# submission2019/cnn-quantization

Hardware: NVIDIA H100
Metric: resnet50_w4a4_images_per_s (higher is better)
Workload: dtype f32

## Files before the change

### cnn-quantization_b200/csrc/fq_bulk.cuh

```cuda
#pragma once
#include <cuda_runtime.h>
#include <stdint.h>

#include "fq_device.cuh"

namespace fqb {

constexpr int kConsumers = kThreads;
constexpr int kBulkThreads = kConsumers + 32;
constexpr int kConsumerWarps = kConsumers / 32;
#ifndef FQB_STAGE_VEC
#define FQB_STAGE_VEC 4
#endif
#ifndef FQB_STAGES
#define FQB_STAGES 6
#endif
#ifndef FQB_BULK_CTAS
#define FQB_BULK_CTAS 1
#endif
constexpr int kBulkCtasPerSm = FQB_BULK_CTAS;
constexpr int kStageVec = FQB_STAGE_VEC;
constexpr int kStages = FQB_STAGES;
constexpr unsigned kStageBytes = kStageVec * kConsumers * 16u;
#ifndef FQB_BULK_SPLIT
// ... 47 lines not shown
  unsigned stride;
  unsigned stage_v;
  unsigned n_stages;
  unsigned unit_stages;
  unsigned units;
  unsigned channels;
  unsigned cv;
};

struct StageMeta {
  unsigned start;
  unsigned count;
  unsigned tag;
  unsigned pad;
};

struct BulkRing {
  alignas(8) unsigned long long full[kStages];
  alignas(8) unsigned long long empty[kStages];
  StageMeta meta[kStages];
  unsigned nstages;
};

struct RingPos {
  unsigned slot, parity, n;
  __device__ __forceinline__ void init(unsigned nstages = kStages) {
    slot = 0;
    parity = 0;
    n = nstages;
  }
  __device__ __forceinline__ void next() {
    if (++slot == n) {
      slot = 0;
      parity ^= 1u;
    }
  }
};

__device__ __forceinline__ void ring_init(BulkRing& r, unsigned nstages = kStages) {
  if (threadIdx.x == 0) {
    r.nstages = nstages;
#pragma unroll
    for (int s = 0; s < kStages; ++s) {
      mbar_init(smem_u32(&r.full[s]), 1u);
      mbar_init(smem_u32(&r.empty[s]), kConsumerWarps);
    }
    mbar_fence_init();
  }
  __syncthreads();
}

struct TicketPlan {
  unsigned nstatic;
  unsigned first, step;
  unsigned dyn_base;
};

constexpr unsigned kPairOffset = kStageBytes / 2u;

__device__ __forceinline__ FlatGeo half_geo(const FlatGeo& g) {
  FlatGeo h = g;
  h.stage_v = (kStageVec / 2u) * g.stride;
  h.n_stages = (g.total_v + h.stage_v - 1u) / h.stage_v;
  h.unit_stages = 2u * g.unit_stages;
  return h;
}

template <bool REV, bool PAIR = false>
__device__ __forceinline__ void produce_phase(const FlatGeo& g, const float4* src, unsigned* counter, const TicketPlan tp,
                                              BulkRing& r, unsigned char* stage_base, RingPos& pos,
                                              const float4* src2 = nullptr) {
  const unsigned total = g.units;
  unsigned k = 0;
  auto fetch = [&]() -> unsigned {
    unsigned long long t;
    if (k < tp.nstatic)
      t = tp.first + static_cast<unsigned long long>(k) * tp.step;
    else
      t = static_cast<unsigned long long>(tp.dyn_base) + atomicAdd(counter, 1u);
    ++k;
    return t < total ? static_cast<unsigned>(t) : 0xffffffffu;
  };
  unsigned cur = fetch();
  unsigned nxt = (cur != 0xffffffffu) ? fetch() : 0xffffffffu;
  while (cur != 0xffffffffu) {
    const unsigned nxt2 = (nxt != 0xffffffffu) ? fetch() : 0xffffffffu;
    const unsigned u = REV ? total - 1u - cur : cur;
    const unsigned g0 = u * g.unit_stages;
    const unsigned g1 = min(g0 + g.unit_stages, g.n_stages);
    for (unsigned i = g0; i < g1; ++i) {
      const unsigned st = REV ? g1 - 1u - (i - g0) : i;
      const unsigned start = st * g.stage_v;
      const unsigned count = min(g.stage_v, g.total_v - start);
      mbar_wait(smem_u32(&r.empty[pos.slot]), pos.parity ^ 1u);
      r.meta[pos.slot].start = start;
      r.meta[pos.slot].count = count;
      r.meta[pos.slot].tag = 0u;
      const unsigned bar = smem_u32(&r.full[pos.slot]);
      mbar_arrive_expect_tx(bar, PAIR ? count * 32u : count * 16u);
      bulk_load(smem_u32(stage_base + pos.slot * kStageBytes), src + start, count * 16u, bar);
      if (PAIR) bulk_load(smem_u32(stage_base + pos.slot * kStageBytes + kPairOffset), src2 + start, count * 16u, bar);
      pos.next();
    }
    cur = nxt;
    nxt = nxt2;
  }
  mbar_wait(smem_u32(&r.empty[pos.slot]), pos.parity ^ 1u);
  r.meta[pos.slot].start = 0u;
  r.meta[pos.slot].count = 0u;
  mbar_arrive(smem_u32(&r.full[pos.slot]));
  pos.next();
}

struct RowsGeo {
  unsigned rows, row_v;
  unsigned stages_per_row;
  unsigned units_per_row;
};

__device__ __forceinline__ RowsGeo half_rows(const FlatGeo& h, const RowsGeo& rg) {
  RowsGeo r = rg;
  r.stages_per_row = (rg.row_v + h.stage_v - 1u) / h.stage_v;
  r.units_per_row = (r.stages_per_row + h.unit_stages - 1u) / h.unit_stages;
  return r;
}

template <bool REV, bool PAIR = false>
__device__ __forceinline__ void produce_rows_phase(const FlatGeo& g, const RowsGeo& rg, const float4* src, unsigned* counter,
                                                   const TicketPlan tp, BulkRing& r, unsigned char* stage_base, RingPos& pos,
                                                   const float4* src2 = nullptr) {
  const unsigned total = g.units;
  unsigned k = 0;
  auto fetch = [&]() -> unsigned {
    unsigned long long t;
    if (k < tp.nstatic)
      t = tp.first + static_cast<unsigned long long>(k) * tp.step;
    else
      t = static_cast<unsigned long long>(tp.dyn_base) + atomicAdd(counter, 1u);
    ++k;
    return t < total ? static_cast<unsigned>(t) : 0xffffffffu;
  };
  unsigned cur = fetch();
  unsigned nxt = (cur != 0xffffffffu) ? fetch() : 0xffffffffu;
  while (cur != 0xffffffffu) {
    const unsigned nxt2 = (nxt != 0xffffffffu) ? fetch() : 0xffffffffu;
    const unsigned u = REV ? total - 1u - cur : cur;
    const unsigned row = u / rg.units_per_row;
    const unsigned part = u - row * rg.units_per_row;
    const unsigned s0 = part * g.unit_stages;
    const unsigned s1 = min(s0 + g.unit_stages, rg.stages_per_row);
    for (unsigned i = s0; i < s1; ++i) {
      const unsigned st = REV ? s1 - 1u - (i - s0) : i;
      const unsigned off = st * g.stage_v;
      const unsigned start = row * rg.row_v + off;
      const unsigned count = min(g.stage_v, rg.row_v - off);
      mbar_wait(smem_u32(&r.empty[pos.slot]), pos.parity ^ 1u);
      r.meta[pos.slot].start = start;
      r.meta[pos.slot].count = count;
      r.meta[pos.slot].tag = row | (i + 1u == s1 ? 0x80000000u : 0u);
      const unsigned bar = smem_u32(&r.full[pos.slot]);
      mbar_arrive_expect_tx(bar, PAIR ? count * 32u : count * 16u);
      bulk_load(smem_u32(stage_base + pos.slot * kStageBytes), src + start, count * 16u, bar);
      if (PAIR) bulk_load(smem_u32(stage_base + pos.slot * kStageBytes + kPairOffset), src2 + start, count * 16u, bar);
      pos.next();
    }
    cur = nxt;
    nxt = nxt2;
  }
  mbar_wait(smem_u32(&r.empty[pos.slot]), pos.parity ^ 1u);
  r.meta[pos.slot].start = 0u;
  r.meta[pos.slot].count = 0u;
  r.meta[pos.slot].tag = 0u;
  mbar_arrive(smem_u32(&r.full[pos.slot]));
  pos.next();
}

struct PoolGeo {
  unsigned h, w;
  unsigned wt;
  unsigned tiles_per_row;
  unsigned row_pairs;
  unsigned tiles;
  unsigned unit_tiles, units;
  unsigned ow;
  unsigned kind;
};

constexpr unsigned kPoolTop = 1u, kPoolLeft = 2u;

__device__ __forceinline__ void produce_pool3_phase(const FlatGeo& g, const PoolGeo& pg, const float4* src, unsigned* counter,
                                                    const TicketPlan tp, BulkRing& r, unsigned char* stage_base, RingPos& pos) {
  const unsigned total = pg.units;
  unsigned k = 0;
  auto fetch = [&]() -> unsigned {
    unsigned long long t;
    if (k < tp.nstatic)
      t = tp.first + static_cast<unsigned long long>(k) * tp.step;
    else
      t = static_cast<unsigned long long>(tp.dyn_base) + atomicAdd(counter, 1u);
    ++k;
    return t < total ? static_cast<unsigned>(t) : 0xffffffffu;
  };
  const unsigned row_v = pg.w * g.cv;
  const unsigned region_v = (2u * pg.wt + 1u) * g.cv;
  const unsigned per_img = pg.row_pairs * pg.tiles_per_row;
  unsigned cur = fetch();
  unsigned nxt = (cur != 0xffffffffu) ? fetch() : 0xffffffffu;
  while (cur != 0xffffffffu) {
    const unsigned nxt2 = (nxt != 0xffffffffu) ? fetch() : 0xffffffffu;
    const unsigned t0 = cur * pg.unit_tiles;
    const unsigned t1 = min(t0 + pg.unit_tiles, pg.tiles);
    for (unsigned tile = t0; tile < t1; ++tile) {
      const unsigned n = tile / per_img;
      const unsigned rem = tile - n * per_img;
      const unsigned oh = rem / pg.tiles_per_row;
      const unsigned wi = rem - oh * pg.tiles_per_row;
      const bool top = oh > 0u, left = wi > 0u;
      const unsigned skip = left ? 0u : g.cv;
      const unsigned count = region_v - skip;
      const unsigned mid = (n * pg.h + 2u * oh) * row_v + (2u * wi * pg.wt) * g.cv - (left ? g.cv : 0u);
      const unsigned o = ((n * pg.row_pairs + oh) * pg.ow + wi * pg.wt) * g.cv;
      mbar_wait(smem_u32(&r.empty[pos.slot]), pos.parity ^ 1u);
      r.meta[pos.slot].start = o;
      r.meta[pos.slot].count = count;
      r.meta[pos.slot].tag = (top ? kPoolTop : 0u) | (left ? kPoolLeft : 0u);
      const unsigned bar = smem_u32(&r.full[pos.slot]);
      mbar_arrive_expect_tx(bar, count * 16u * (top ? 3u : 2u));
      const unsigned dst = smem_u32(stage_base + pos.slot * kStageBytes) + skip * 16u;
      if (top) bulk_load(dst, src + mid - row_v, count * 16u, bar);
      bulk_load(dst + region_v * 16u, src + mid, count * 16u, bar);
      bulk_load(dst + 2u * region_v * 16u, src + mid + row_v, count * 16u, bar);
      pos.next();
    }
    cur = nxt;
    nxt = nxt2;
  }
  mbar_wait(smem_u32(&r.empty[pos.slot]), pos.parity ^ 1u);
  r.meta[pos.slot].start = 0u;
  r.meta[pos.slot].count = 0u;
  r.meta[pos.slot].tag = 0u;
  mbar_arrive(smem_u32(&r.full[pos.slot]));
  pos.next();
}

template <typename Acc>
__device__ __forceinline__ void consume_pool3_phase(const FlatGeo& g, const PoolGeo& pg, BulkRing& r, const unsigned char* stage_base,
                                                    RingPos& pos, Acc& acc) {
  const unsigned t = threadIdx.x;
  const bool lane0 = (t & 31u) == 0u;
  const bool mine = t < pg.wt * g.cv;
  const unsigned j = t / g.cv, col = t - j * g.cv;
  const unsigned region = (2u * pg.wt + 1u) * g.cv * 16u;
  const unsigned my = smem_u32(stage_base) + ((2u * j) * g.cv + col) * 16u;
  const unsigned nxt = g.cv * 16u;
  for (;;) {
    mbar_wait(smem_u32(&r.full[pos.slot]), pos.parity);
    const StageMeta m = r.meta[pos.slot];
    if (m.count != 0u && mine) {
      const unsigned addr = my + pos.slot * kStageBytes;
      const bool first = (j != 0u) || (m.tag & kPoolLeft);
      acc.pool_begin();
#pragma unroll
      for (int dy = 0; dy < 3; ++dy) {
        if (dy == 0 && !(m.tag & kPoolTop)) continue;
        const unsigned row = addr + dy * region;
        float4 v;
        if (first) {
          lds_vec(row, v);
          acc.pool_tap(v);
        }
        lds_vec(row + nxt, v);
        acc.pool_tap(v);
        lds_vec(row + 2u * nxt, v);
        acc.pool_tap(v);
      }
      acc.pool_end(m.start + t);
    }
    __syncwarp();
    if (lane0) mbar_arrive(smem_u32(&r.empty[pos.slot]));
    pos.next();
    if (m.count == 0u) break;
  }
}

__device__ __forceinline__ void produce_pool_phase(const FlatGeo& g, const PoolGeo& pg, const float4* src, unsigned* counter,
                                                   const TicketPlan tp, BulkRing& r, unsigned char* stage_base, RingPos& pos) {
  const unsigned total = pg.units;
  unsigned k = 0;
  auto fetch = [&]() -> unsigned {
    unsigned long long t;
    if (k < tp.nstatic)
      t = tp.first + static_cast<unsigned long long>(k) * tp.step;
    else
      t = static_cast<unsigned long long>(tp.dyn_base) + atomicAdd(counter, 1u);
    ++k;
    return t < total ? static_cast<unsigned>(t) : 0xffffffffu;
  };
  const unsigned row_v = pg.w * g.cv;
  const unsigned count = pg.wt * g.cv;
  const unsigned per_img = pg.row_pairs * pg.tiles_per_row;
  unsigned cur = fetch();
  unsigned nxt = (cur != 0xffffffffu) ? fetch() : 0xffffffffu;
  while (cur != 0xffffffffu) {
    const unsigned nxt2 = (nxt != 0xffffffffu) ? fetch() : 0xffffffffu;
    const unsigned t0 = cur * pg.unit_tiles;
    const unsigned t1 = min(t0 + pg.unit_tiles, pg.tiles);
    for (unsigned tile = t0; tile < t1; ++tile) {
      const unsigned n = tile / per_img;
      const unsigned rem = tile - n * per_img;
      const unsigned hp = rem / pg.tiles_per_row;
      const unsigned wi = rem - hp * pg.tiles_per_row;
      const unsigned a = (n * pg.h + 2u * hp) * row_v + wi * count;
      const unsigned o = ((n * pg.row_pairs + hp) * pg.ow + wi * (pg.wt / 2u)) * g.cv;
      mbar_wait(smem_u32(&r.empty[pos.slot]), pos.parity ^ 1u);
      r.meta[pos.slot].start = o;
      r.meta[pos.slot].count = count;
      r.meta[pos.slot].tag = 0u;
      const unsigned bar = smem_u32(&r.full[pos.slot]);
      mbar_arrive_expect_tx(bar, count * 32u);
      bulk_load(smem_u32(stage_base + pos.slot * kStageBytes), src + a, count * 16u, bar);
      bulk_load(smem_u32(stage_base + pos.slot * kStageBytes + kPairOffset), src + a + row_v, count * 16u, bar);
      pos.next();
    }
    cur = nxt;
    nxt = nxt2;
  }
  mbar_wait(smem_u32(&r.empty[pos.slot]), pos.parity ^ 1u);
  r.meta[pos.slot].start = 0u;
  r.meta[pos.slot].count = 0u;
  r.meta[pos.slot].tag = 0u;
  mbar_arrive(smem_u32(&r.full[pos.slot]));
  pos.next();
}

template <typename Acc>
__device__ __forceinline__ void consume_pool_phase(const FlatGeo& g, const PoolGeo& pg, BulkRing& r, const unsigned char* stage_base,
                                                   RingPos& pos, Acc& acc) {
  const unsigned t = threadIdx.x;
  const bool lane0 = (t & 31u) == 0u;
  const bool mine = t < (pg.wt / 2u) * g.cv;
  const unsigned j = t / g.cv, col = t - j * g.cv;
  const unsigned my = smem_u32(stage_base) + ((2u * j) * g.cv + col) * 16u;
  const unsigned nxt = g.cv * 16u;
  for (;;) {
    mbar_wait(smem_u32(&r.full[pos.slot]), pos.parity);
    const StageMeta m = r.meta[pos.slot];
    if (m.count != 0u && mine) {
      const unsigned addr = my + pos.slot * kStageBytes;
      float4 a0, a1, b0, b1;
      lds_vec(addr, a0);
      lds_vec(addr + nxt, a1);
      lds_vec(addr + kPairOffset, b0);
      lds_vec(addr + kPairOffset + nxt, b1);
      acc.pooled(a0, a1, b0, b1, m.start + t);
    }
    __syncwarp();
    if (lane0) mbar_arrive(smem_u32(&r.empty[pos.slot]));
    pos.next();
    if (m.count == 0u) break;
  }
}

template <typename Acc>
__device__ __forceinline__ void consume_phase(const FlatGeo& g, BulkRing& r, const unsigned char* stage_base, RingPos& pos,
                                              Acc& acc) {
  const unsigned t = threadIdx.x;
  const bool lane0 = (t & 31u) == 0u;
  const unsigned my = smem_u32(stage_base) + t * 16u;
  const unsigned step = g.stride * 16u;
  for (;;) {
    mbar_wait(smem_u32(&r.full[pos.slot]), pos.parity);
    const StageMeta m = r.meta[pos.slot];
    const unsigned addr = my + pos.slot * kStageBytes;
    if (m.count == g.stage_v) {
      if (t < g.stride) {
        float4 x[kStageVec];
#pragma unroll
        for (int i = 0; i < kStageVec; ++i) lds_vec(addr + i * step, x[i]);
#pragma unroll
        for (int i = 0; i < kStageVec; ++i) acc.consume(x[i], m.start + t + i * g.stride);
      }
    } else if (m.count != 0u) {
#pragma unroll
      for (int i = 0; i < kStageVec; ++i) {
        const unsigned idx = t + i * g.stride;
        if (t < g.stride && idx < m.count) {
          float4 x;
          lds_vec(addr + i * step, x);
          acc.consume(x, m.start + idx);
        }
      }
    }
    acc.stage_end(m);
    __syncwarp();
    if (lane0) mbar_arrive(smem_u32(&r.empty[pos.slot]));
    pos.next();
    if (m.count == 0u) break;
  }
}

template <typename Acc>
__device__ __forceinline__ void consume_pair_phase(const FlatGeo& g, BulkRing& r, const unsigned char* stage_base, RingPos& pos,
                                                   Acc& acc) {
  static_assert(kStageVec % 2u == 0u, "a pair stage is split in two halves");
  constexpr int kHalf = kStageVec / 2;
  const unsigned t = threadIdx.x;
  const bool lane0 = (t & 31u) == 0u;
  const unsigned my = smem_u32(stage_base) + t * 16u;
// ... 38 lines not shown
```

### cnn-quantization_b200/csrc/fq_cl.cuh

```cuda
#pragma once

namespace fqb {

__device__ __forceinline__ unsigned enc_ordered(float x) {
  const unsigned b = __float_as_uint(x);
  return (b & 0x80000000u) ? ~b : (b | 0x80000000u);
}
__device__ __forceinline__ float dec_ordered(unsigned e) {
  return __uint_as_float((e & 0x80000000u) ? (e & 0x7fffffffu) : ~e);
}

constexpr unsigned kAccU = 2u * kMaxNhwcChannels;
constexpr unsigned kAccD = 3u * kMaxNhwcChannels;

struct ClView {
  unsigned* amin_inv;
  unsigned* amax;
  double* asum;
  double* asq;
  double* aabs;
};
__device__ __forceinline__ ClView cl_view(const FusedArgs& A, unsigned bank) {
  ClView v;
  v.amin_inv = A.amin_inv + bank * kAccU;
// ... 635 lines not shown
      produce_phase<false>(g, src, &A.sync->unit_counter[0], all, ring, stages, pos);
      if (DEV) {
        mbar_wait(smem_u32(&phase_go[0]), 0u);
        if (solver_in_s2 && blockIdx.x == 0) mbar_wait(smem_u32(&solver_done), 0u);
        produce_phase<true>(g, src, &A.sync->unit_counter[1], solver_in_s2 ? no0 : all, ring, stages, pos);
      }
      if (!A.stats_only) {
        mbar_wait(smem_u32(&phase_go[1]), 0u);
        if (A.pool.tiles && A.pool.kind == 3u)
          produce_pool3_phase(g, A.pool, src, &A.sync->unit_counter[2], all, ring, stages, pos);
        else if (A.pool.tiles)
          produce_pool_phase(g, A.pool, src, &A.sync->unit_counter[2], all, ring, stages, pos);
        else if (A.residual)
          produce_phase<!DEV, true>(half_geo(g), src, &A.sync->unit_counter[2], all, ring, stages, pos,
                                    reinterpret_cast<const float4*>(A.residual));
        else
          produce_phase<!DEV>(g, src, &A.sync->unit_counter[2], all, ring, stages, pos);
      }
    }
    return;
  }

  const unsigned t = threadIdx.x;
  const bool active = t < g.stride;
  const bool direct = cv == g.stride;
  const unsigned col = active ? t % cv : 0u;
  const unsigned c0 = 4u * col;
  const double n = A.n_per_group;
  const ClView acc = cl_view(A, bank);
  const unsigned rep = A.nhwc_rep;
  const unsigned rep_base = (blockIdx.x % rep) * C;
  unsigned epoch = 0;
  if (blockIdx.x == 0) stamp(A, 0);

  if (blockIdx.x == gridDim.x - 1u) {
    const ClView other = cl_view(A, bank ^ 1u);
    uint4* zu = reinterpret_cast<uint4*>(other.amin_inv);
    uint4* zd = reinterpret_cast<uint4*>(other.asum);
    const uint4 z = make_uint4(0u, 0u, 0u, 0u);
    for (unsigned i = t; i < kAccU / 4u; i += kConsumers) zu[i] = z;
    for (unsigned i = t; i < kAccD / 2u; i += kConsumers) zd[i] = z;
  }

  ClCtx cx;
  cx.g = &g;
  cx.ring = &ring;
  cx.stages = stages;
  cx.cbuf = cbuf;
  cx.pos.init(nstages);
  cx.acc = acc;
  cx.rep_base = rep_base;
  cx.c0 = c0;
  cx.active = active;
  float kshift[4];
  cl_phase_s1(A, cx, kshift);
  if (t == 0) mbar_arrive(smem_u32(&phase_go[DEV ? 0 : 1]));
  if (blockIdx.x == 0) stamp(A, 1);
  grid_barrier_cl(A.sync, epoch);
  if (blockIdx.x == 0) stamp(A, 4);

  float mean[4];
  if (direct) {
#pragma unroll
    for (int i = 0; i < 4; ++i)
      mean[i] = static_cast<float>(cl_mean(acc, rep, C, c0 + i, kshift[i], (A.bias && active) ? __ldg(A.bias + c0 + i) : 0.f, n));
  } else {
    for (unsigned c = t; c < C; c += kConsumers)
      tab_mean[c] = static_cast<float>(cl_mean(acc, rep, C, c, ld_tensor(A.in + c), A.bias ? __ldg(A.bias + c) : 0.f, n));
    consumer_sync();
#pragma unroll
    for (int i = 0; i < 4; ++i) mean[i] = tab_mean[c0 + i];
  }

  if (alloc && !aux_needs_b && blockIdx.x == 0) {
    cl_solve_aux(A, acc, lsm, tag, false, !solver_in_s2);
    stamp(A, 12);
    if (t == 0) mbar_arrive(smem_u32(&solver_done));
  }

  if constexpr (DEV) {
    cl_phase_s2(A, cx, mean);
    if (t == 0) mbar_arrive(smem_u32(&phase_go[1]));
    if (blockIdx.x == 0) stamp(A, 5);
    grid_barrier_cl(A.sync, epoch);
    if (blockIdx.x == 0) stamp(A, 8);
    if (aux_needs_b && blockIdx.x == 0) cl_solve_aux(A, acc, lsm, tag, true, true);
  }
  if (alloc && !solver_in_s2) {
    if (t == 0)
      while (ld_acquire_u32(&A.sync->aux_ready) != tag) __nanosleep(40);
    consumer_sync();
  }

  LeafParam lp[4];
  const bool do_export = A.out_stats != nullptr && blockIdx.x == 0;
  if (direct) {
#pragma unroll
    for (int i = 0; i < 4; ++i) lp[i] = cl_channel_param<LEAF, DEV>(A, acc, rep, C, c0 + i, mean[i], n, alloc, do_export && active);
  } else {
    LeafParam* tab_lp = reinterpret_cast<LeafParam*>(cbuf);
    consumer_sync();
    for (unsigned c = t; c < C; c += kConsumers) tab_lp[c] = cl_channel_param<LEAF, DEV>(A, acc, rep, C, c, tab_mean[c], n, alloc, do_export);
    consumer_sync();
#pragma unroll
    for (int i = 0; i < 4; ++i) lp[i] = tab_lp[c0 + i];
  }
  if (blockIdx.x == 0) stamp(A, 7);

  if (!A.stats_only) {
    cl_phase_apply<LEAF, HIST>(A, cx, lp, hist);
    if (blockIdx.x == 0) stamp(A, 9);
  }
  grid_exit_cl(A.sync);
}

template <bool GRID>
struct ClGiven {
  const FusedArgs& A;
  LeafParam q[4];
  float r[4], bias[4];
  bool fast;
  template <bool FAST>
  __device__ __forceinline__ void one(const float4& v, unsigned off) {
    const float x[4] = {v.x, v.y, v.z, v.w};
    float y[4], gq[4];
#pragma unroll
    for (int i = 0; i < 4; ++i) {
      Divisor dv;
      dv.s = q[i].a;
      dv.r = r[i];
      dv.fast = FAST;
      y[i] = leaf_apply<FQB200_LEAF_TORCH, FAST>(__fadd_rn(x[i], bias[i]), q[i], dv, 0.f, gq[i]);
    }
    st_tensor(reinterpret_cast<float4*>(A.out) + off, make_float4(y[0], y[1], y[2], y[3]));
    if (GRID) st_tensor(reinterpret_cast<float4*>(A.grid_out) + off, make_float4(gq[0], gq[1], gq[2], gq[3]));
  }
  __device__ __forceinline__ void consume(const float4& v, unsigned off) {
    if (fast)
      one<true>(v, off);
    else
      one<false>(v, off);
  }
  __device__ __forceinline__ void stage_end(const StageMeta&) {}
};

template <bool GRID>
__global__ void __launch_bounds__(kBulkThreads, kBulkCtasPerSm) fq_cl_given_kernel(const __grid_constant__ FusedArgs A) {
  extern __shared__ __align__(128) unsigned char fq_dyn[];
  __shared__ BulkRing ring;
  const FlatGeo& g = A.flat;
  ring_init(ring);
  if (threadIdx.x >= kConsumers) {
    if (threadIdx.x == kConsumers) {
      RingPos pos;
      pos.init();
      const TicketPlan tp = {0xffffffffu, blockIdx.x, gridDim.x, 0u};
      produce_phase<false>(g, reinterpret_cast<const float4*>(A.in), nullptr, tp, ring, fq_dyn, pos);
    }
    return;
  }
  const unsigned t = threadIdx.x;
  const bool active = t < g.stride;
  const unsigned c0 = active ? 4u * (t % g.cv) : 0u;
  ClGiven<GRID> ap{A};
  ap.fast = true;
#pragma unroll
  for (int i = 0; i < 4; ++i) {
// ... 544 lines not shown
```

### cnn-quantization_b200/csrc/fqb200.cu

```cuda
#include <cuda_runtime.h>
#include <math.h>
#include <stdint.h>
#include <stdio.h>
#include <stdlib.h>
#include <string.h>

#include "../../include/fqb200.h"
#include "fq_device.cuh"
#include "fq_bulk.cuh"

namespace fqb {

__constant__ float kGaus[9] = {0.f, 1.24f, 1.71f, 2.15f, 2.55f, 2.93f, 3.28f, 3.61f, 3.92f};
__constant__ float kGausPos[9] = {0.f, 1.71f, 2.15f, 2.55f, 2.93f, 3.28f, 3.61f, 3.92f, 4.2f};
__constant__ float kLaplace[9] = {1.05f, 1.86f, 2.83f, 3.89f, 5.03f, 6.2f, 7.41f, 8.64f, 9.89f};
__constant__ float kLaplacePos[9] = {1.86f, 2.83f, 3.89f, 5.02f, 6.2f, 7.41f, 8.64f, 9.89f, 11.16f};
constexpr int kTable = 101;
__constant__ double kOmegaTable[kTable];
__constant__ double kAlphaTable[kTable];

enum : int { FLAG_PASSTHROUGH = 1, FLAG_TRUE_ZERO = 2, FLAG_RELU = 4 };

struct alignas(16) LeafParam {
  float a, b, c;
// ... 1258 lines not shown
      continue;
    }
    if (worst < 1) {
      d.rc = FQB200_ERR_CUDA;
      snprintf(d.err, sizeof(d.err), "channels-last kernel does not fit on an SM");
      return;
    }
    d.resident_cl[hist] = sms * worst;
  }
  {
    int n = 0;
    const void* fn = reinterpret_cast<const void*>(fqb::fq_cl_bca_kernel);
    e = cudaFuncSetAttribute(fn, cudaFuncAttributeMaxDynamicSharedMemorySize, static_cast<int>(cl_smem(false)));
    if (e == cudaSuccess) e = cudaOccupancyMaxActiveBlocksPerMultiprocessor(&n, fn, fqb::kBulkThreads, cl_smem(false));
    if (e != cudaSuccess || n < 1) return bad("bias-correction kernel setup", e);
    d.resident_bca = sms * n;
  }
  {
    int n = 0;
    const void* fn = reinterpret_cast<const void*>(fqb::fq_rows_kernel);
    e = cudaFuncSetAttribute(fn, cudaFuncAttributeMaxDynamicSharedMemorySize, static_cast<int>(cl_given_smem()));
    if (e == cudaSuccess) e = cudaOccupancyMaxActiveBlocksPerMultiprocessor(&n, fn, fqb::kBulkThreads, cl_given_smem());
    if (e != cudaSuccess || n < 1) return bad("row kernel setup", e);
    d.resident_rows = sms * n;
  }
  const void* given[4] = {reinterpret_cast<const void*>(fqb::fq_given_kernel<4, FQB200_LEAF_TORCH, false>),
                          reinterpret_cast<const void*>(fqb::fq_given_kernel<4, FQB200_LEAF_TORCH, true>),
                          reinterpret_cast<const void*>(fqb::fq_cl_given_kernel<false>),
                          reinterpret_cast<const void*>(fqb::fq_cl_given_kernel<true>)};
  for (int i = 0; i < 4; ++i) {
    e = cudaFuncSetAttribute(given[i], cudaFuncAttributeMaxDynamicSharedMemorySize,
                             static_cast<int>(i < 2 ? dyn_smem(4) : cl_given_smem()));
    if (e != cudaSuccess) return bad("given-parameter kernel setup", e);
  }
  e = cudaFuncSetAttribute(reinterpret_cast<const void*>(fqb::fq_cl_given_fused_kernel), cudaFuncAttributeMaxDynamicSharedMemorySize,
                           static_cast<int>(cl_given_smem()));
  if (e != cudaSuccess) return bad("given-parameter fused kernel setup", e);
  const void* leafb[2] = {reinterpret_cast<const void*>(fqb::fq_leaf_bulk_kernel<false>),
                          reinterpret_cast<const void*>(fqb::fq_leaf_bulk_kernel<true>)};
  for (int i = 0; i < 2; ++i) {
    e = cudaFuncSetAttribute(leafb[i], cudaFuncAttributeMaxDynamicSharedMemorySize, static_cast<int>(cl_given_smem()));
    if (e != cudaSuccess) return bad("a1 bulk kernel setup", e);
  }
  double om[fqb::kTable], al[fqb::kTable];
  om[0] = 0.0;
  al[0] = 0.0;
  const double lo[5] = {0.01, 0.1, 1, 10, 100}, hi[5] = {0.1, 1, 10, 100, 1000};
  for (int dcd = 0; dcd < 5; ++dcd)
    for (int k = 0; k < 20; ++k) {
      const double w = lo[dcd] + (hi[dcd] - lo[dcd]) * k / 20.0;
      om[1 + dcd * 20 + k] = w;
      al[1 + dcd * 20 + k] = laplace_opt_alpha(w);
    }
  e = cudaMemcpyToSymbol(fqb::kOmegaTable, om, sizeof(om));
  if (e == cudaSuccess) e = cudaMemcpyToSymbol(fqb::kAlphaTable, al, sizeof(al));
  if (e != cudaSuccess) return bad("table upload", e);
  d.sms = sms;
  d.resident = sms * per_sm;
}

int get_device(DeviceInfo** out) {
  int dev = 0;
  cudaError_t e = cudaGetDevice(&dev);
  if (e != cudaSuccess) return fail(FQB200_ERR_CUDA, "cudaGetDevice: %s", cudaGetErrorString(e));
  if (dev < 0 || dev >= kMaxDevices) return fail(FQB200_ERR_UNSUPPORTED, "device index out of range%s");
  std::call_once(g_dev_once[dev], init_device, dev);
  DeviceInfo& d = g_dev[dev];
  if (d.rc != FQB200_OK) return fail(d.rc, "device set-up failed: %s", d.err);
  *out = &d;
  return FQB200_OK;
}

struct Plan {
  fqb::Geometry geo;
  fqb::FlatGeo flat;
  int vec;
  int mode;
  int grid;
};

bool aligned16(const void* p) { return (reinterpret_cast<uintptr_t>(p) & 15u) == 0; }

constexpr uint64_t kUnitsPerCta = 8;

int make_plan(int64_t outer, int64_t groups, int64_t inner, bool can_vec, bool allow_bundle, int max_ctas, Plan* pl) {
  if (outer <= 0 || groups <= 0 || inner <= 0) return fail(FQB200_ERR_INVALID, "non-positive tensor extent%s");
  if (groups > 0x3fffffffLL || outer > 0x7fffffffLL || inner > 0x7fffffffLL * 4LL)
    return fail(FQB200_ERR_UNSUPPORTED, "tensor extent exceeds 2^31%s");
  int vec = (can_vec && inner % 4 == 0) ? 4 : 1;
  int mode = vec;
  uint64_t bundle = 1;
  if (vec == 1 && can_vec && allow_bundle && inner >= 4) {
    const uint64_t b = (inner % 2 == 0) ? 2 : 4;
    const uint64_t row_v = b * static_cast<uint64_t>(inner) / 4;
    if (groups % b == 0 && row_v <= static_cast<uint64_t>(fqb::kThreads)) {
      bundle = b;
      vec = 4;
      mode = 8;
    }
  }
  const uint64_t G = static_cast<uint64_t>(groups) / bundle;
  const uint64_t inner_v = bundle * static_cast<uint64_t>(inner) / vec;
  if (inner_v > 0xffffffffULL) return fail(FQB200_ERR_UNSUPPORTED, "row too long%s");
  const uint64_t stride = (mode == 8) ? (fqb::kThreads / inner_v) * inner_v : fqb::kThreads;
  const uint64_t group_v = static_cast<uint64_t>(outer) * inner_v;
  const uint64_t total_v = group_v * G;
  if (total_v >= (1ULL << 32)) return fail(FQB200_ERR_UNSUPPORTED, "tensors of 2^32 vectors (64 GB) and more are not supported%s");
  const uint64_t ctas = static_cast<uint64_t>(max_ctas);
  const uint64_t min_unit_v = static_cast<uint64_t>(fqb::kRingDepth) * stride;
  uint64_t parts = (kUnitsPerCta * ctas + G - 1) / G;
  const uint64_t max_parts = group_v / min_unit_v > 0 ? group_v / min_unit_v : 1;
  if (parts > max_parts) parts = max_parts;
  if (parts < 1) parts = 1;
  while ((group_v + parts - 1) / parts >= 0x7fffffffULL) ++parts;
  uint64_t part_v = (group_v + parts - 1) / parts;
  if (mode == 8) part_v = (part_v + inner_v - 1) / inner_v * inner_v;
  parts = (group_v + part_v - 1) / part_v;
  if (parts * G >= 0xfffffff0ULL) return fail(FQB200_ERR_UNSUPPORTED, "too many work units%s");
  const uint64_t units = parts * G;
  unsigned lanes = 32;
  while (lanes > 1 && (static_cast<uint64_t>(fqb::kThreads / lanes) < static_cast<uint64_t>(groups) || (lanes >> 1) >= parts)) lanes >>= 1;
  fqb::Geometry& g = pl->geo;
  g.groups = static_cast<unsigned>(G);
  g.channels = static_cast<unsigned>(groups);
  g.bundle = static_cast<unsigned>(bundle);
  g.stride = static_cast<unsigned>(stride);
  g.parts = static_cast<unsigned>(parts);
  g.units = static_cast<unsigned>(units);
  g.inner_v = static_cast<unsigned>(inner_v);
  g.step_q = static_cast<unsigned>(stride / inner_v);
  g.step_r = static_cast<unsigned>(stride % inner_v);
  g.red_lanes = lanes;
  g.part_v = static_cast<unsigned>(part_v);
  g.group_v = group_v;
  g.row_pitch = G * inner_v;
  pl->vec = vec;
  pl->mode = mode;
  pl->grid = static_cast<int>(units < ctas ? units : ctas);
  return FQB200_OK;
}

bool flat_eligible(int64_t channels) { return channels % 4 == 0 && channels / 4 >= 1 && channels / 4 <= fqb::kConsumers; }

int make_plan_flat(uint64_t elems, int64_t channels, int max_ctas, Plan* pl) {
  if (elems == 0 || elems % 4 != 0) return fail(FQB200_ERR_UNSUPPORTED, "flat stream needs a multiple of 4 elements%s");
  const uint64_t total_v = elems / 4;
  if (total_v >= (1ULL << 32)) return fail(FQB200_ERR_UNSUPPORTED, "tensors of 2^32 vectors (64 GB) and more are not supported%s");
  const uint64_t cv = channels > 0 ? static_cast<uint64_t>(channels) / 4 : 1;
  if (channels > 0 && !flat_eligible(channels)) return fail(FQB200_ERR_UNSUPPORTED, "channels-last needs C %% 4 == 0 and C <= 2048%s");
  const uint64_t stride = (fqb::kConsumers / cv) * cv;
  const uint64_t stage_v = static_cast<uint64_t>(fqb::kStageVec) * stride;
  const uint64_t n_stages = (total_v + stage_v - 1) / stage_v;
  const uint64_t ctas = static_cast<uint64_t>(max_ctas);
  uint64_t unit_stages = n_stages / (kUnitsPerCta * ctas);
  if (unit_stages < 2) unit_stages = 2;
  if (unit_stages > 64) unit_stages = 64;
  const uint64_t units = (n_stages + unit_stages - 1) / unit_stages;
  fqb::FlatGeo& g = pl->flat;
  g.total_v = static_cast<unsigned>(total_v);
  g.stride = static_cast<unsigned>(stride);
  g.stage_v = static_cast<unsigned>(stage_v);
  g.n_stages = static_cast<unsigned>(n_stages);
  g.unit_stages = static_cast<unsigned>(unit_stages);
  g.units = static_cast<unsigned>(units);
  g.channels = static_cast<unsigned>(channels > 0 ? channels : 0);
  g.cv = static_cast<unsigned>(cv);
  memset(&pl->geo, 0, sizeof(pl->geo));
  pl->geo.channels = g.channels;
  pl->vec = 4;
  pl->mode = 2;
  pl->grid = static_cast<int>(units < ctas ? units : ctas);
  return FQB200_OK;
}

int make_plan_rows(uint64_t rows, uint64_t row_elems, int64_t channels, int max_ctas, Plan* pl, fqb::RowsGeo* rg) {
  if (rows == 0 || row_elems == 0 || row_elems % 4 != 0 || rows > fqb::kMaxNhwcChannels)
    return fail(FQB200_ERR_UNSUPPORTED, "row stream needs rows <= 4096 of a multiple of 4 elements%s");
  const uint64_t row_v = row_elems / 4;
  if (rows * row_v >= (1ULL << 32)) return fail(FQB200_ERR_UNSUPPORTED, "tensors of 2^32 vectors (64 GB) and more are not supported%s");
  const uint64_t cv = channels > 0 ? static_cast<uint64_t>(channels) / 4 : 1;
  if (channels > 0 && (!flat_eligible(channels) || row_v % cv != 0)) return fail(FQB200_ERR_UNSUPPORTED, "bias period does not fit the rows%s");
  const uint64_t stride = (fqb::kConsumers / cv) * cv;
  const uint64_t stage_v = static_cast<uint64_t>(fqb::kStageVec) * stride;
  const uint64_t spr = (row_v + stage_v - 1) / stage_v;
  const uint64_t ctas = static_cast<uint64_t>(max_ctas);
  uint64_t unit_stages = rows * spr / (kUnitsPerCta * ctas);
  if (unit_stages < 1) unit_stages = 1;
  if (unit_stages > 64) unit_stages = 64;
  if (unit_stages > spr) unit_stages = spr;
  const uint64_t upr = (spr + unit_stages - 1) / unit_stages;
  const uint64_t units = rows * upr;
  if (units >= 0xfffffff0ULL) return fail(FQB200_ERR_UNSUPPORTED, "too many work units%s");
  fqb::FlatGeo& g = pl->flat;
  g.total_v = static_cast<unsigned>(rows * row_v);
  g.stride = static_cast<unsigned>(stride);
  g.stage_v = static_cast<unsigned>(stage_v);
  g.n_stages = static_cast<unsigned>(rows * spr);
  g.unit_stages = static_cast<unsigned>(unit_stages);
  g.units = static_cast<unsigned>(units);
  g.channels = static_cast<unsigned>(channels > 0 ? channels : 0);
  g.cv = static_cast<unsigned>(cv);
  rg->rows = static_cast<unsigned>(rows);
  rg->row_v = static_cast<unsigned>(row_v);
  rg->stages_per_row = static_cast<unsigned>(spr);
  rg->units_per_row = static_cast<unsigned>(upr);
  memset(&pl->geo, 0, sizeof(pl->geo));
  pl->geo.channels = static_cast<unsigned>(rows);
  pl->vec = 4;
  pl->mode = 3;
  pl->grid = static_cast<int>(units < ctas ? units : ctas);
  return FQB200_OK;
}

bool rows_supported(const fqb200_desc* d, bool can_vec) {
  if (d->leaf != FQB200_LEAF_COMPILED || d->range_mode != FQB200_RANGE_MINMAX || d->bias_corr || d->var_corr || d->channels_last ||
      d->out_hist || !can_vec || d->outer != 1 || d->inner % 4 != 0 || d->groups > static_cast<int64_t>(fqb::kMaxNhwcChannels))
    return false;
  if (!(d->scope == FQB200_SCOPE_GROUP_MEAN || d->scope == FQB200_SCOPE_TENSOR || d->groups == 1)) return false;
  if (d->bias) {
    if (d->bias_period >= 0) return false;
    const int64_t c = -d->bias_period;
    if (!flat_eligible(c) || d->inner % c != 0) return false;
  }
  return true;
}

size_t align_up(size_t v, size_t a) { return (v + a - 1) / a * a; }

size_t kld_workspace(int64_t rows, int num_bins) {
  return align_up(static_cast<size_t>(rows) * 4, 256) + static_cast<size_t>(rows) * static_cast<size_t>(num_bins) * 4;
}

size_t sumsq_workspace(int64_t rows, int64_t row_len) {
  const unsigned long long chunk = fqb::sumsq_chunk(static_cast<unsigned long long>(row_len));
  const unsigned long long chunks = (static_cast<unsigned long long>(row_len) + chunk - 1) / chunk;
  return chunks > 1 ? static_cast<size_t>(rows) * static_cast<size_t>(chunks) * 8 : 0;
}

unsigned long long cliperr_units_per_group(int64_t outer, int64_t inner, int channels_last) {
// ... 106 lines not shown
  if (d->leaf < FQB200_LEAF_TORCH || d->leaf > FQB200_LEAF_MIDTREAD) return fail(FQB200_ERR_INVALID, "bad leaf%s");
  if (d->leaf != FQB200_LEAF_MIDTREAD && (d->num_bits < 1 || d->num_bits > 8))
    return fail(FQB200_ERR_INVALID, "num_bits must be in 1..8%s");
  if (d->scope != FQB200_SCOPE_GROUP && (d->range_mode != FQB200_RANGE_MINMAX || d->leaf == FQB200_LEAF_MIDTREAD))
    return fail(FQB200_ERR_UNSUPPORTED, "group-mean / tensor scopes are defined for min/max ranges only%s");
  if (d->bit_alloc && !(d->bit_alloc_target > 0.f)) return fail(FQB200_ERR_INVALID, "bit_alloc_target must be > 0%s");
  if ((d->bias_corr || d->var_corr) && d->scope == FQB200_SCOPE_GROUP_MEAN)
    return fail(FQB200_ERR_UNSUPPORTED, "weight correction is per row (scope GROUP or TENSOR)%s");
  return FQB200_OK;
}

unsigned pool_tile_width(int kind, int64_t w, const fqb::FlatGeo& f) {
  const unsigned cv = f.cv, stage_v = fqb::kStageVec * fqb::kConsumers;
  if (kind == 2) {
    for (int64_t cand = w; cand >= 2; cand -= 2)
      if (w % cand == 0 && static_cast<uint64_t>(cand) * cv <= stage_v / 2u && static_cast<uint64_t>(cand / 2) * cv <= f.stride)
        return static_cast<unsigned>(cand);
  } else {
    const int64_t ow = w / 2;
    for (int64_t cand = ow; cand >= 1; --cand)
      if (ow % cand == 0 && 3ull * static_cast<uint64_t>(2 * cand + 1) * cv <= stage_v && static_cast<uint64_t>(cand) * cv <= f.stride)
        return static_cast<unsigned>(cand);
  }
  return 0;
}

struct FusedPlan {
  Plan pl;
  fqb::FusedArgs A;
  uint64_t slots;
  size_t workspace;
  const void* kernel;
  unsigned block;
  size_t smem;
  bool coop;
  const char* name;
};

int plan_fused(const fqb200_desc* d, bool can_vec, const DeviceInfo& r, FusedPlan* fp) {
  memset(fp, 0, sizeof(*fp));
  Plan& pl = fp->pl;
  fqb::FusedArgs& A = fp->A;
  if (d->outer <= 0 || d->groups <= 0 || d->inner <= 0) return fail(FQB200_ERR_INVALID, "non-positive tensor extent%s");
  if (d->bias && d->bias_period == 0 && d->scope == FQB200_SCOPE_GROUP_MEAN)
    return fail(FQB200_ERR_UNSUPPORTED, "a per-group bias needs groups = channels (scope GROUP or TENSOR); use bias_period%s");
  const bool given = d->range_mode == FQB200_RANGE_GIVEN;
  int rc;
  if (d->channels_last) {
    if (!can_vec || d->scope != FQB200_SCOPE_GROUP || d->leaf == FQB200_LEAF_COMPILED || d->bias_corr || d->var_corr ||
        d->bias_period > 0 || !flat_eligible(d->groups))
      return fail(FQB200_ERR_UNSUPPORTED, "channels_last: per-channel torch / mid-tread leaves on 16-byte aligned tensors, C %% 4 == 0, C <= 2048%s");
    rc = make_plan_flat(static_cast<uint64_t>(d->outer) * d->groups * d->inner, d->groups,
                        given ? r.resident_cl[0] * 2 : r.resident_cl[d->out_hist ? 1 : 0], &pl);
  } else if (rows_supported(d, can_vec)) {
    rc = make_plan_rows(static_cast<uint64_t>(d->groups), static_cast<uint64_t>(d->inner), d->bias ? -d->bias_period : 0,
                        r.resident_rows, &pl, &A.rows);
  } else if (d->bias && d->bias_period < 0) {
    return fail(FQB200_ERR_UNSUPPORTED, "a channel-fastest bias (bias_period < 0) needs the per-sample / per-tensor min-max layout%s");
  } else {
    rc = make_plan(d->outer, d->groups, d->inner, can_vec, !(d->bias_corr || d->var_corr), r.resident, &pl);
  }
  if (rc != FQB200_OK) return rc;
  if ((d->residual_stats || d->residual_bias) && !d->residual)
    return fail(FQB200_ERR_INVALID, "residual_stats / residual_bias without a residual%s");
  if (d->residual_bias && !d->residual_stats)
    return fail(FQB200_ERR_INVALID, "residual_bias needs residual_stats (a bias on a plain addend can be folded by the caller)%s");
  if (d->residual && ((!d->channels_last && pl.mode != 3) || d->stats_only || !aligned16(d->residual)))
    return fail(FQB200_ERR_UNSUPPORTED, "residual: channels-last or per-sample / per-tensor min-max apply launches, 16-byte aligned%s");
  if (d->pool) {
    const bool rows_cl = pl.mode == 3 && d->bias && d->bias_period < 0;
    if ((d->pool != 2 && d->pool != 3) || !(d->channels_last || rows_cl) || d->stats_only || d->residual || d->out_hist || !d->pool_out ||
        !aligned16(d->pool_out))
      return fail(FQB200_ERR_UNSUPPORTED, "pool: 2 (2x2 stride 2) or 3 (3x3 stride 2 padding 1) on channels-last apply launches without residual / histogram, 16-byte aligned pool_out%s");
    const int64_t h = d->pool_h, w = d->pool_w;
    const int64_t hw = rows_cl ? d->inner / -d->bias_period : d->inner;
    const int64_t images = rows_cl ? d->groups : d->outer;
    if (h < 2 || w < 2 || w % 2 != 0 || h * w != hw || (d->pool == 3 && h % 2 != 0))
      return fail(FQB200_ERR_UNSUPPORTED, "pool: pool_h * pool_w must be H * W of the tensor, W even (3x3: H even too)%s");
    const unsigned wt = pool_tile_width(d->pool, w, pl.flat);
    if (!wt) return fail(FQB200_ERR_UNSUPPORTED, "pool: no tile width fits%s");
    const int64_t tiles_per_row = (d->pool == 2 ? w : w / 2) / wt;
    const uint64_t tiles = static_cast<uint64_t>(images) * static_cast<uint64_t>(h / 2) * static_cast<uint64_t>(tiles_per_row);
    if (tiles >= 0xfffffff0ull) return fail(FQB200_ERR_UNSUPPORTED, "pool: too many tiles%s");
    uint64_t unit_tiles = tiles / (kUnitsPerCta * static_cast<uint64_t>(pl.grid));
    if (unit_tiles < 2) unit_tiles = 2;
    if (unit_tiles > 64) unit_tiles = 64;
    A.pool.h = static_cast<unsigned>(h);
    A.pool.w = static_cast<unsigned>(w);
    A.pool.wt = wt;
    A.pool.tiles_per_row = static_cast<unsigned>(tiles_per_row);
    A.pool.row_pairs = static_cast<unsigned>(h / 2);
    A.pool.tiles = static_cast<unsigned>(tiles);
    A.pool.unit_tiles = static_cast<unsigned>(unit_tiles);
    A.pool.units = static_cast<unsigned>((tiles + unit_tiles - 1) / unit_tiles);
    A.pool.ow = static_cast<unsigned>(w / 2);
    A.pool.kind = static_cast<unsigned>(d->pool);
    A.pool_out = d->pool_out;
  }
  A.hist_bins = d->out_hist ? (d->hist_bins > 0 ? d->hist_bins : 256) : 0;
  if (d->out_hist && d->leaf != FQB200_LEAF_TORCH && !d->channels_last)
    return fail(FQB200_ERR_UNSUPPORTED, "out_hist: torch leaf, or the mid-tread leaf on channels-last tensors%s");
  if (d->out_hist && (A.hist_bins > static_cast<int>(fqb::kHistWords) || (!d->channels_last && A.hist_bins != 256)))
    return fail(FQB200_ERR_UNSUPPORTED, "hist_bins: 256 (default), up to 8192 on channels-last tensors%s");
  A.geo = pl.geo;
  A.flat = pl.flat;
  A.scope = d->scope;
  A.range_mode = d->range_mode;
  A.leaf = d->leaf;
  A.num_bits = d->num_bits;
  A.positive = d->positive;
  A.solve_f64 = d->solve_f64;
  A.clip_k = d->clip_k;
  A.bit_alloc = d->bit_alloc;
  A.prior = d->bit_alloc_prior;
  A.ba_round = d->bit_alloc_round;
  A.ba_target = d->bit_alloc_target;
  A.mt_target = d->mt_target;
  A.mt_clip = d->mt_clip;
  A.bias_corr = d->bias_corr;
  A.var_corr = d->var_corr;
  A.stats_only = d->stats_only;
  A.relu_passthrough = d->relu_passthrough;
  A.residual = d->residual;
  A.residual_relu = d->residual_relu;
  A.residual_stats = d->residual_stats;
  A.residual_bias = d->residual_bias;
  A.out_stats = d->out_stats;
  A.bias = d->bias;
  A.hist = d->out_hist;
  A.hist_offset = d->hist_offset;
  A.hist_clamped = d->out_hist_clamped;
  A.dbg = d->debug_stamps;
  fp->block = fqb::kBulkThreads;
  fp->coop = !given;
  if (given) {
    A.g_delta = d->given_delta;
    A.g_offset = d->given_offset;
    A.g_bits = d->given_bits;
    A.given_per_group = 1;
    fp->kernel = reinterpret_cast<const void*>(fqb::fq_cl_given_fused_kernel);
    fp->smem = cl_given_smem();
    fp->name = "fq_cl_given_fused_kernel";
    return FQB200_OK;
  }
  if (pl.mode == 3) {
    if (d->scope == FQB200_SCOPE_GROUP) A.scope = FQB200_SCOPE_TENSOR;
    A.n_per_group = static_cast<double>(d->inner);
    fp->kernel = reinterpret_cast<const void*>(fqb::fq_rows_kernel);
    fp->smem = cl_given_smem();
    fp->name = "fq_rows_kernel";
  } else {
    if (d->bias && d->bias_period > 0) {
      const uint64_t pv = static_cast<uint64_t>(d->bias_period) / pl.vec;
      if (pl.mode != 4 || d->leaf != FQB200_LEAF_COMPILED || d->range_mode != FQB200_RANGE_MINMAX || d->bias_corr || d->var_corr ||
          d->stats_only || d->bias_period % pl.vec != 0 || d->inner % d->bias_period != 0 || pv == 0 ||
          static_cast<uint64_t>(pl.geo.inner_v) * pv >= (1ull << 40) || pl.geo.inner_v >= (1u << 24))
        return fail(FQB200_ERR_UNSUPPORTED, "bias_period does not fit this layout%s");
      A.bias_magic = ((1ull << 40) + pv - 1) / pv;
    }
    A.inner = static_cast<unsigned>(d->inner);
    A.n_per_group = static_cast<double>(d->outer) * static_cast<double>(d->inner);
    const bool alloc = d->bit_alloc && d->num_bits <= 4 && d->scope == FQB200_SCOPE_GROUP && d->leaf != FQB200_LEAF_MIDTREAD;
    if (pl.mode == 2) {
      const unsigned rep = fqb::kMaxNhwcChannels / static_cast<unsigned>(d->groups);
      A.nhwc_rep = rep < 1u ? 1u : (rep > 8u ? 8u : rep);
      A.need_dev = d->range_mode == FQB200_RANGE_LAPLACE || (d->leaf == FQB200_LEAF_MIDTREAD && d->mt_clip) ||
                   (alloc && d->bit_alloc_prior == FQB200_PRIOR_B) || d->stats_only || d->out_stats != nullptr;
      fp->kernel = cl_kernel_ptr(d->leaf, A.need_dev != 0, d->out_hist != nullptr);
      fp->smem = cl_smem(d->out_hist != nullptr);
// ... 582 lines not shown
```

Baseline: 8912.

## Fix work-unit size to two stages, drop ticket prefetch, overlap barrier with param solve

The producer loops no longer fetch work tickets two units ahead; they fetch only the next ticket. The unit size for flat and pool scheduling becomes a fixed two stages or tiles instead of scaling with tensor size. Separately, the channels-last grid barrier is split into arrive and wait, and thread 0 speculatively computes the channel parameter while waiting. Smaller units improve load balance but cost more atomic ticket fetches, and the shallower prefetch exposes more atomic latency.

New measurement: 9040, median of 6. 1.01x the previous value.

```diff
diff --git a/cnn-quantization_b200/csrc/fq_bulk.cuh b/cnn-quantization_b200/csrc/fq_bulk.cuh
--- a/cnn-quantization_b200/csrc/fq_bulk.cuh
+++ b/cnn-quantization_b200/csrc/fq_bulk.cuh
@@ -153,9 +153,8 @@
     return t < total ? static_cast<unsigned>(t) : 0xffffffffu;
   };
   unsigned cur = fetch();
-  unsigned nxt = (cur != 0xffffffffu) ? fetch() : 0xffffffffu;
   while (cur != 0xffffffffu) {
-    const unsigned nxt2 = (nxt != 0xffffffffu) ? fetch() : 0xffffffffu;
+    const unsigned nxt = fetch();
     const unsigned u = REV ? total - 1u - cur : cur;
     const unsigned g0 = u * g.unit_stages;
     const unsigned g1 = min(g0 + g.unit_stages, g.n_stages);
@@ -174,7 +173,6 @@
       pos.next();
     }
     cur = nxt;
-    nxt = nxt2;
   }
   mbar_wait(smem_u32(&r.empty[pos.slot]), pos.parity ^ 1u);
   r.meta[pos.slot].start = 0u;
@@ -212,9 +210,8 @@
     return t < total ? static_cast<unsigned>(t) : 0xffffffffu;
   };
   unsigned cur = fetch();
-  unsigned nxt = (cur != 0xffffffffu) ? fetch() : 0xffffffffu;
   while (cur != 0xffffffffu) {
-    const unsigned nxt2 = (nxt != 0xffffffffu) ? fetch() : 0xffffffffu;
+    const unsigned nxt = fetch();
     const unsigned u = REV ? total - 1u - cur : cur;
     const unsigned row = u / rg.units_per_row;
     const unsigned part = u - row * rg.units_per_row;
@@ -236,7 +233,6 @@
       pos.next();
     }
     cur = nxt;
-    nxt = nxt2;
   }
   mbar_wait(smem_u32(&r.empty[pos.slot]), pos.parity ^ 1u);
   r.meta[pos.slot].start = 0u;
@@ -276,9 +272,8 @@
   const unsigned region_v = (2u * pg.wt + 1u) * g.cv;
   const unsigned per_img = pg.row_pairs * pg.tiles_per_row;
   unsigned cur = fetch();
-  unsigned nxt = (cur != 0xffffffffu) ? fetch() : 0xffffffffu;
   while (cur != 0xffffffffu) {
-    const unsigned nxt2 = (nxt != 0xffffffffu) ? fetch() : 0xffffffffu;
+    const unsigned nxt = fetch();
     const unsigned t0 = cur * pg.unit_tiles;
     const unsigned t1 = min(t0 + pg.unit_tiles, pg.tiles);
     for (unsigned tile = t0; tile < t1; ++tile) {
@@ -304,7 +299,6 @@
       pos.next();
     }
     cur = nxt;
-    nxt = nxt2;
   }
   mbar_wait(smem_u32(&r.empty[pos.slot]), pos.parity ^ 1u);
   r.meta[pos.slot].start = 0u;
@@ -371,9 +365,8 @@
   const unsigned count = pg.wt * g.cv;
   const unsigned per_img = pg.row_pairs * pg.tiles_per_row;
   unsigned cur = fetch();
-  unsigned nxt = (cur != 0xffffffffu) ? fetch() : 0xffffffffu;
   while (cur != 0xffffffffu) {
-    const unsigned nxt2 = (nxt != 0xffffffffu) ? fetch() : 0xffffffffu;
+    const unsigned nxt = fetch();
     const unsigned t0 = cur * pg.unit_tiles;
     const unsigned t1 = min(t0 + pg.unit_tiles, pg.tiles);
     for (unsigned tile = t0; tile < t1; ++tile) {
@@ -394,7 +387,6 @@
       pos.next();
     }
     cur = nxt;
-    nxt = nxt2;
   }
   mbar_wait(smem_u32(&r.empty[pos.slot]), pos.parity ^ 1u);
   r.meta[pos.slot].start = 0u;
diff --git a/cnn-quantization_b200/csrc/fq_cl.cuh b/cnn-quantization_b200/csrc/fq_cl.cuh
--- a/cnn-quantization_b200/csrc/fq_cl.cuh
+++ b/cnn-quantization_b200/csrc/fq_cl.cuh
@@ -741,7 +741,12 @@
     cl_phase_s2(A, cx, mean);
     if (t == 0) mbar_arrive(smem_u32(&phase_go[1]));
     if (blockIdx.x == 0) stamp(A, 5);
-    grid_barrier_cl(A.sync, epoch);
+    grid_arrive_cl(A.sync, epoch);
+    if (t == 0 && ld_acquire_u32(&A.sync->release) < epoch) {
+      const LeafParam w = cl_channel_param<LEAF, DEV>(A, acc, rep, C, c0, mean[0], n, alloc, false);
+      asm volatile("" ::"f"(w.a), "f"(w.b), "f"(w.c), "r"(w.flags));
+    }
+    grid_wait_cl(A.sync, epoch);
     if (blockIdx.x == 0) stamp(A, 8);
     if (aux_needs_b && blockIdx.x == 0) cl_solve_aux(A, acc, lsm, tag, true, true);
   }
diff --git a/cnn-quantization_b200/csrc/fqb200.cu b/cnn-quantization_b200/csrc/fqb200.cu
--- a/cnn-quantization_b200/csrc/fqb200.cu
+++ b/cnn-quantization_b200/csrc/fqb200.cu
@@ -1364,6 +1364,7 @@
 bool aligned16(const void* p) { return (reinterpret_cast<uintptr_t>(p) & 15u) == 0; }
 
 constexpr uint64_t kUnitsPerCta = 8;
+constexpr uint64_t kUnitStages = 2;
 
 int make_plan(int64_t outer, int64_t groups, int64_t inner, bool can_vec, bool allow_bundle, int max_ctas, Plan* pl) {
   if (outer <= 0 || groups <= 0 || inner <= 0) return fail(FQB200_ERR_INVALID, "non-positive tensor extent%s");
@@ -1434,9 +1435,7 @@
   const uint64_t stage_v = static_cast<uint64_t>(fqb::kStageVec) * stride;
   const uint64_t n_stages = (total_v + stage_v - 1) / stage_v;
   const uint64_t ctas = static_cast<uint64_t>(max_ctas);
-  uint64_t unit_stages = n_stages / (kUnitsPerCta * ctas);
-  if (unit_stages < 2) unit_stages = 2;
-  if (unit_stages > 64) unit_stages = 64;
+  const uint64_t unit_stages = kUnitStages;
   const uint64_t units = (n_stages + unit_stages - 1) / unit_stages;
   fqb::FlatGeo& g = pl->flat;
   g.total_v = static_cast<unsigned>(total_v);
@@ -1709,9 +1708,7 @@
     const int64_t tiles_per_row = (d->pool == 2 ? w : w / 2) / wt;
     const uint64_t tiles = static_cast<uint64_t>(images) * static_cast<uint64_t>(h / 2) * static_cast<uint64_t>(tiles_per_row);
     if (tiles >= 0xfffffff0ull) return fail(FQB200_ERR_UNSUPPORTED, "pool: too many tiles%s");
-    uint64_t unit_tiles = tiles / (kUnitsPerCta * static_cast<uint64_t>(pl.grid));
-    if (unit_tiles < 2) unit_tiles = 2;
-    if (unit_tiles > 64) unit_tiles = 64;
+    const uint64_t unit_tiles = kUnitStages;
     A.pool.h = static_cast<unsigned>(h);
     A.pool.w = static_cast<unsigned>(w);
     A.pool.wt = wt;
```
